# vpc-ccg/tksm

Measured on AMD Instinct MI355X. Metric: sequenced reads/s, higher is better.
Workload: dtype u8; 1 GPU; Bulk molecules, Badread error+qual model (nanopore2020, identity 84,99,5.5), 24 x 128 Mb random genome, FASTQ; kind=bulk, mean_len=1000, length_distribution=normal(1000, 200), compute_qual=True, contexts_in_flight_per_gpu=3

## Files before the change

### tksm_amd/csrc/kernels.h

```cpp
#pragma once
#include <hip/hip_runtime.h>
#include <stdint.h>

namespace tk {

constexpr uint32_t NO_BLOCK = 0xFFFFFFFFu;
constexpr int BLOCK_SHIFT = 12;
constexpr int WAVES_PER_WG = 4;

struct RefView {
    const uint32_t* packed;
    const uint32_t* blocktab;
    const uint8_t* pool;
    const uint64_t* contigs;
    uint32_t n_contigs;
};

struct BatchView {
    const uint32_t* reads;
    const uint32_t* intervals;
    const uint32_t* mods;
    const uint64_t* literals;
    const uint8_t* litpool;
    const uint32_t* ids;
    const uint8_t* idpool;
    uint64_t n_reads;
    uint32_t n_literals;
};

struct ErrModelView {
    int type, k, max_alts;
    int alt0_noop;
    int uniform_nalts;
    const uint32_t* cdf;
    const uint64_t* alts;
    const uint8_t* nalts;
    const uint2* pself2;
    const uint32_t* cdf32;
    const uint4* pseg;
    const uint32_t* pt0;
    const uint4* pt0b;
    const uint4* alts_enc;
};

struct QsModelView {
    int n_slots, kmer_size;
    const uint64_t* keys;
    const uint32_t* row_off;
    const uint32_t* row_cnt;
    const uint32_t* cdf_pool;
    const uint8_t* q_pool;
    const uint4* ent;
    const uint2* pairs;
    const uint8_t* guide;
    int guide_direct;
};

struct IdentView {
    int constant;
    double value;
    const double* qtab;
};

struct TailView {
    int n_lx, n_ly;
    double ratio;
    const double* lx;
    const double* ly;
    const double* cdf;
};
struct TailChain {
    double cum[16];
    uint32_t bases;
    uint32_t pad;
};

struct SimParams {
    uint64_t seed, first_read, stride;
    int mode, compute_q, fastq, quirk_perfect;
    int lcap;
    int ncap;
    int trace_words;
    int s_lcap, s_ncap;
    int ablate;
    int cap_num, cap_den, cap_add;
};

struct SimBuffers {
    const uint32_t* raw_len;
    const uint64_t* slot_off;
    uint8_t* scratch;
    uint32_t* out_len;
    double* identity;
    uint64_t* rec_len;
    uint32_t* status;
    uint32_t* trace;
    unsigned long long* work_counter;
    int32_t* istats;
    double* dstats;
    uint8_t* full_pool; unsigned long long full_pool_bytes; unsigned long long* full_pool_used;
    const uint32_t* tail_len;
    const TailChain* tail_chain;
    uint8_t* big_scratch; size_t big_per_wave; unsigned long long* big_trace;
    const uint32_t* read_list;
    uint64_t n_work;
};

struct ReadState {
    double errors, target, est;
    int32_t change_count;
    uint32_t n_base, aln_no;
    int16_t resume_src, resume_j;
    uint8_t stage;
    uint8_t pending, slow, early;
    int32_t st_draws, st_aligns;
    uint32_t job;
    int32_t raw_len;
    uint32_t res_mt, res_cols, res_fail, pad3;
};

struct RangeGeo {
    uint64_t trace_off;
    uint64_t jc_off;
    uint64_t popd_off;
    uint64_t unused;
    uint32_t tstride;
    uint32_t cw;
    uint32_t ncap;
    uint32_t pad;
};

enum Counter {
    CNT_JOBS = 0,
    CNT_DEFERRED = 1,
    CNT_SLOW = 2,
    CNT_FULL_ROWS = 3,
    CNT_EXIT = 4,
    CNT_REDO_JOBS = 8,
    CNT_REDO_WAVES = 9,
    CNT_REDO_LIST = 10,
    CNT_FAIL = 12,
    CNT_FAIL_OR = 13,
    CNT_FAIL_LAST = 14,
    CNT_FAIL_NM = 15,
    CNT_FAIL_REASON = 16,
    CNT_FAIL_QJOB = 24,
    CNT_FAIL_LIST = 25,
    CNT_EARLY_SLOW = 26,
    CNT_EARLY = 27,
    CNT_WORDS = 32
};
enum ExitCause { EXIT_BAND_LOOP = 0, EXIT_SHIFT_LOOP = 1, EXIT_SHIFT_ERR = 2, EXIT_BAND_ERR = 3 };
enum FailBit { FAIL_QUEUE = 0, FAIL_NOROW = 1, FAIL_SHIFT31 = 3, FAIL_SHIFT14 = 4, FAIL_END_CELL = 5, FAIL_WALK = 6 };

struct FastBuffers {
    ReadState* state;
    const uint32_t* row64;
    uint8_t* st_frag;
    uint16_t* st_nb;
    unsigned long long* st_fplanes;
    uint32_t* st_frag2;
    uint32_t* job_meta;
    uint8_t* job_popd;
    void* trace;
    uint32_t* redo_list;
    void* trace_full;
    uint32_t full_rows, full_tg;
    uint32_t full_cl;
    uint32_t* counters;
    uint32_t* job_cnt;
    uint32_t rs, n_ranges;
    const uint32_t* prev_meta; const uint8_t* prev_popd;
    const uint32_t* prefix;
    const uint32_t* base_cur; const uint32_t* base_prev;
    const RangeGeo* geo_cur; const RangeGeo* geo_prev;
    uint32_t* slow_list;
    uint32_t* early_hist;
    uint2* early_list;
    uint32_t* early_slow;
    uint2* defer_list;
    uint32_t* defer_cnt;
    int defer_len;
};

hipError_t launch_pack(const uint8_t* ascii, uint64_t n, uint64_t gstart, uint32_t* packed, uint32_t* blockflag,
                       hipStream_t s);
hipError_t launch_fill_pool(const uint8_t* ascii, uint64_t n, uint64_t gstart, const uint32_t* blocktab,
                            uint8_t* pool, hipStream_t s);
hipError_t launch_read_lengths(const BatchView& b, const RefView& r, int k, int cap_num, int cap_den, int cap_add,
                               const uint32_t* tail_len, uint32_t* raw_len, uint64_t* slot_cap, uint32_t* status, hipStream_t s);
hipError_t launch_tail_lengths(const BatchView& B, const RefView& R, const TailView& T, uint64_t seed, uint64_t first_read,
                               uint64_t stride, uint32_t* tail_len, hipStream_t s);
hipError_t launch_simulate(const BatchView& b, const RefView& r, const ErrModelView& em, const QsModelView& qm,
                           const IdentView& im, const SimParams& p, const SimBuffers& o, int n_wgs,
                           int waves_per_wg, hipStream_t s);
size_t simulate_big_bytes(int lcap, int ncap);
hipError_t launch_simulate_big(const BatchView& b, const RefView& r, const ErrModelView& em, const QsModelView& qm,
                               const IdentView& im, const SimParams& p, const SimBuffers& o, int n_waves, hipStream_t s);
hipError_t launch_init(const BatchView& b, const RefView& r, const ErrModelView& em, const IdentView& im, const SimParams& p,
                       const SimBuffers& o, const FastBuffers& fb, int waves_per_wg, hipStream_t s);
int err_lds_bytes(int lcap, int ncap, int waves_per_wg, bool state_in_hbm);
int loop_lds_words(int lcap);
hipError_t launch_loopw(const ErrModelView& em, const SimParams& p, const FastBuffers& fb, const uint32_t* order, uint32_t begin,
                        uint32_t count, int lcap, int from_jobs, uint32_t c0, uint32_t c1, hipStream_t s);
hipError_t launch_tail(const ErrModelView& em, const SimParams& p, const FastBuffers& fb, const uint32_t* order, uint32_t begin,
                        uint32_t count, int lcap, int from_jobs, uint32_t c0, uint32_t c1, int wcap, hipStream_t s);
size_t tail_lds_bytes(int lcap);
hipError_t launch_mark_early(const FastBuffers& fb, const uint32_t* order, uint64_t n_reads, int k, uint32_t min_bin, hipStream_t s);
hipError_t launch_tail_early(const ErrModelView& em, const SimParams& p, const FastBuffers& fb, uint32_t max_count, int lcap, int wcap, hipStream_t s);
hipError_t launch_merge_early_slow(const FastBuffers& fb, hipStream_t s);
hipError_t launch_loop(const ErrModelView& em, const SimParams& p, const FastBuffers& fb, const uint32_t* order, uint32_t begin,
                       uint32_t count, int lcap, int from_jobs, uint32_t c0, uint32_t c1, hipStream_t s);
hipError_t launch_err(const BatchView& b, const ErrModelView& em, const QsModelView& qm, const SimParams& p, const SimBuffers& o,
                      const FastBuffers& fb, const uint32_t* order, uint32_t begin, uint32_t count, int lds_lcap, int lds_ncap,
                      int from_jobs, uint32_t c0, uint32_t c1, int waves_per_wg, bool state_in_hbm, hipStream_t s);
hipError_t launch_qjobs(const FastBuffers& fb, int k, uint32_t count, hipStream_t s);
hipError_t launch_round_reset(const FastBuffers& fb, hipStream_t s);
hipError_t launch_collect_unfinished(const FastBuffers& fb, uint64_t n_reads, hipStream_t s);
hipError_t launch_alnf(const SimParams& p, const FastBuffers& fb, const SimBuffers& o, uint32_t n_jobs, bool full_only, int mode, hipStream_t s);
hipError_t launch_perfect_lengths(const BatchView& b, const RefView& r, const SimParams& p, const SimBuffers& o, hipStream_t s);
hipError_t launch_perfect(const BatchView& b, const RefView& r, const SimParams& p, const SimBuffers& o, const uint64_t* rec_off, uint8_t* records,
                          uint32_t max_raw, int n_cus, hipStream_t s);
hipError_t launch_emit(const BatchView& b, const SimParams& p, const SimBuffers& o, const uint64_t* rec_off,
                       uint8_t* records, hipStream_t s);
hipError_t launch_interleave_lens(int n_ranks, const uint64_t* const* offsets, const uint64_t* n_per_rank,
                                  uint64_t n_total, uint64_t* lens, hipStream_t s);
hipError_t launch_interleave_copy(int n_ranks, const uint8_t* const* streams, const uint64_t* const* offsets,
                                  uint64_t n_total, const uint64_t* dst_off, uint8_t* dst, hipStream_t s);
size_t scan_temp_bytes(uint64_t n);
hipError_t launch_scan(const uint64_t* in, uint64_t* out, uint64_t n, void* temp, size_t temp_bytes, hipStream_t s);
hipError_t launch_sum_u32(const uint32_t* in, uint64_t n, unsigned long long* out, hipStream_t s);
int simulate_lds_bytes(int lcap, int ncap, int waves_per_wg);
int simulate_max_wgs(int lds_bytes);

}
```

### tksm_amd/csrc/kernels.hip

```cpp
#include "kernels.h"
#include "loop_filter.h"
#include <type_traits>

namespace tk {

#define DEV __device__ __forceinline__

constexpr int BIG = 1 << 28;
DEV bool is_inf(int v) { return v >= (1 << 27); }

struct Ph4 { uint32_t x, y, z, w; };
enum { ST_ID = 0, ST_PAD = 1, ST_IDENT = 2, ST_DRAW = 3, ST_ALNPOS = 4, ST_QUAL = 5, ST_TAIL = 6 };

DEV Ph4 philox(uint64_t seed, uint64_t read, uint32_t stream, uint32_t n) {
    uint32_t c0 = (uint32_t)read, c1 = (uint32_t)(read >> 32), c2 = stream, c3 = n;
    uint32_t k0 = (uint32_t)seed, k1 = (uint32_t)(seed >> 32);
#pragma unroll
    for (int r = 0; r < 10; r++) {
        const unsigned long long p0 = (unsigned long long)0xD2511F53u * c0, p1 = (unsigned long long)0xCD9E8D57u * c2;
        const uint32_t h0 = (uint32_t)(p0 >> 32), l0 = (uint32_t)p0, h1 = (uint32_t)(p1 >> 32), l1 = (uint32_t)p1;
        uint32_t n0 = h1 ^ c1 ^ k0, n2 = h0 ^ c3 ^ k1;
        c0 = n0; c1 = l1; c2 = n2; c3 = l0;
        k0 += 0x9E3779B9u; k1 += 0xBB67AE85u;
    }
    return Ph4{c0, c1, c2, c3};
}

DEV uint8_t base_char(int code) { return (uint8_t)((0x54474341u >> (8 * (code & 3))) & 0xff); }
DEV int code_of(uint8_t c) { return c == 'A' ? 0 : c == 'C' ? 1 : c == 'G' ? 2 : c == 'T' ? 3 : -1; }
DEV uint8_t upper(uint8_t c) { return (c >= 'a' && c <= 'z') ? (uint8_t)(c - 32) : c; }
DEV uint8_t comp(uint8_t c) {
    return c == 'A' ? 'T' : c == 'C' ? 'G' : c == 'G' ? 'C' : c == 'T' ? 'A' : c;
}

template <int CTRL, int ROW_MASK> DEV int dpp_mov(int old, int src) { return __builtin_amdgcn_update_dpp(old, src, CTRL, ROW_MASK, 0xf, false); }
constexpr int DPP_WAVE_SHL1 = 0x130, DPP_WAVE_SHR1 = 0x138;
#define TKSM_DPP_SCAN(OP, IDENT, x)                         \
    x = OP(x, dpp_mov<0x111, 0xf>(IDENT, x));               \
    x = OP(x, dpp_mov<0x112, 0xf>(IDENT, x));               \
    x = OP(x, dpp_mov<0x114, 0xf>(IDENT, x));               \
    x = OP(x, dpp_mov<0x118, 0xf>(IDENT, x));               \
    x = OP(x, dpp_mov<0x142, 0xa>(IDENT, x));               \
    x = OP(x, dpp_mov<0x143, 0xc>(IDENT, x));
DEV int scan_min_incl(int x, int) { TKSM_DPP_SCAN(min, 0x7fffffff, x) return x; }
DEV int scan_max_incl(int x, int) { TKSM_DPP_SCAN(max, (int)0x80000000, x) return x; }
DEV int add_i32(int a, int b) { return a + b; }
DEV int scan_add_incl(int x, int) { TKSM_DPP_SCAN(add_i32, 0, x) return x; }
DEV uint32_t scan_umax_incl(uint32_t x) {
#define TKSM_UMAX_STEP(C, R) x = max(x, (uint32_t)dpp_mov<C, R>(0, (int)x));
    TKSM_UMAX_STEP(0x111, 0xf) TKSM_UMAX_STEP(0x112, 0xf) TKSM_UMAX_STEP(0x114, 0xf) TKSM_UMAX_STEP(0x118, 0xf) TKSM_UMAX_STEP(0x142, 0xa) TKSM_UMAX_STEP(0x143, 0xc)
#undef TKSM_UMAX_STEP
    return x;
}
DEV int prefix_small(int v, int& total) {
    const unsigned long long b0 = __ballot(v & 1), b1 = __ballot(v & 2), b2 = __ballot(v & 4);
    const int e0 = (int)__builtin_amdgcn_mbcnt_hi((uint32_t)(b0 >> 32), __builtin_amdgcn_mbcnt_lo((uint32_t)b0, 0u));
    const int e1 = (int)__builtin_amdgcn_mbcnt_hi((uint32_t)(b1 >> 32), __builtin_amdgcn_mbcnt_lo((uint32_t)b1, 0u));
    const int e2 = (int)__builtin_amdgcn_mbcnt_hi((uint32_t)(b2 >> 32), __builtin_amdgcn_mbcnt_lo((uint32_t)b2, 0u));
    total = __popcll(b0) + 2 * __popcll(b1) + 4 * __popcll(b2);
    return e0 + 2 * e1 + 4 * e2;
}

DEV void wave_sync() {
    __builtin_amdgcn_fence(__ATOMIC_RELEASE, "wavefront");
    __builtin_amdgcn_wave_barrier();
    __builtin_amdgcn_fence(__ATOMIC_ACQUIRE, "wavefront");
}

DEV uint32_t lo32(unsigned long long v) { return (uint32_t)v; }
DEV uint32_t hi32(unsigned long long v) { return (uint32_t)(v >> 32); }
DEV unsigned long long mk64(uint32_t hi, uint32_t lo) { return ((unsigned long long)hi << 32) | lo; }
DEV uint32_t alignbit(uint32_t hi, uint32_t lo, uint32_t s) { return __builtin_amdgcn_alignbit(hi, lo, s); }
constexpr uint32_t TA = 0xF0u, TB = 0xCCu, TC = 0xAAu;
#define BOOL3(expr) ((uint32_t)((expr) & 0xFFu))
template <uint32_t TT> DEV uint32_t bool3(uint32_t x, uint32_t y, uint32_t z) { return __builtin_amdgcn_bitop3_b32(x, y, z, TT); }
template <uint32_t TT> DEV unsigned long long bool3(unsigned long long x, unsigned long long y, unsigned long long z) {
    return mk64(bool3<TT>(hi32(x), hi32(y), hi32(z)), bool3<TT>(lo32(x), lo32(y), lo32(z)));
}
DEV unsigned long long funnel128(unsigned long long x0, unsigned long long x1, int s) {
    const bool a = (s & 32) != 0;
    const uint32_t b = (uint32_t)s & 31u;
    const uint32_t y0 = a ? hi32(x0) : lo32(x0), y1 = a ? lo32(x1) : hi32(x0), y2 = a ? hi32(x1) : lo32(x1);
    return mk64(alignbit(y2, y1, b), alignbit(y1, y0, b));
}

DEV double sqrt_inrange(double x) {
    const double y = __builtin_amdgcn_rsq(x);
    double g = x * y, h = 0.5 * y;
    const double r = __builtin_fma(-h, g, 0.5);
    g = __builtin_fma(g, r, g); h = __builtin_fma(h, r, h);
    double d = __builtin_fma(-g, g, x);
    g = __builtin_fma(d, h, g);
    d = __builtin_fma(-g, g, x);
    return __builtin_fma(d, h, g);
}
DEV double rcp_refined(double b) {
    double y = __builtin_amdgcn_rcp(b);
    double r = __builtin_fma(-b, y, 1.0);
    y = __builtin_fma(y, r, y);
    r = __builtin_fma(-b, y, 1.0);
    return __builtin_fma(y, r, y);
}
DEV double div_inrange(double a, double b, double yb) {
    const double q = a * yb;
    const double r = __builtin_fma(-b, q, a);
    return __builtin_fma(r, yb, q);
}

DEV uint8_t ref_base(const RefView& R, uint64_t g) {
    uint32_t ex = R.blocktab[g >> BLOCK_SHIFT];
    if (ex != NO_BLOCK) return R.pool[((uint64_t)ex << BLOCK_SHIFT) + (g & ((1u << BLOCK_SHIFT) - 1))];
    uint32_t w = R.packed[g >> 4];
    return base_char((int)(w >> ((g & 15) * 2)));
}

DEV int slot_len(uint32_t code) { return code ? (int)((code >> 12) & 7) : 1; }
DEV uint8_t slot_sym(uint32_t code, int x, uint8_t orig) {
    if (!code) return orig;
    if ((int)((code >> 10) & 3) == x + 1) return orig;
    return base_char((int)(code >> (2 * x)));
}

__global__ void k_pack(const uint8_t* __restrict__ ascii, uint64_t n, uint64_t gstart, uint32_t* __restrict__ packed,
                       uint32_t* __restrict__ blockflag) {
    uint64_t w = (uint64_t)blockIdx.x * blockDim.x + threadIdx.x;
    uint64_t nw = (n + 15) >> 4;
    for (; w < nw; w += (uint64_t)gridDim.x * blockDim.x) {
        uint64_t b0 = w << 4;
        uint32_t word = 0; bool exc = false;
        if (b0 + 16 <= n && ((uintptr_t)(ascii + b0) & 15) == 0) {
            uint4 v = *reinterpret_cast<const uint4*>(ascii + b0);
            uint32_t q[4] = {v.x, v.y, v.z, v.w};
#pragma unroll
            for (int i = 0; i < 16; i++) {
                int c = code_of(upper((uint8_t)(q[i >> 2] >> (8 * (i & 3)))));
                exc |= c < 0; word |= (uint32_t)(c & 3) << (2 * i);
            }
        } else {
            for (int i = 0; i < 16 && b0 + i < n; i++) {
                int c = code_of(upper(ascii[b0 + i]));
                exc |= c < 0; word |= (uint32_t)(c & 3) << (2 * i);
            }
        }
        packed[(gstart >> 4) + w] = word;
        if (exc) blockflag[(gstart + b0) >> BLOCK_SHIFT] = 1;
    }
}

__global__ void k_fill_pool(const uint8_t* __restrict__ ascii, uint64_t n, uint64_t gstart,
                            const uint32_t* __restrict__ blocktab, uint8_t* __restrict__ pool) {
    uint64_t i = (uint64_t)blockIdx.x * blockDim.x + threadIdx.x;
    for (; i < n; i += (uint64_t)gridDim.x * blockDim.x) {
        uint64_t g = gstart + i;
        uint32_t ex = blocktab[g >> BLOCK_SHIFT];
// ... 656 lines not shown
        }
    }
    if (a == 16) {
        uint4 v[4];
#pragma unroll
        for (int q = 0; q < 4; q++) v[q] = c4[4 + q];
#pragma unroll
        for (int q = 0; q < 4; q++) {
            a += !(w < v[q].x) ? 1 : 0; a += !(w < v[q].y) ? 1 : 0; a += !(w < v[q].z) ? 1 : 0; a += !(w < v[q].w) ? 1 : 0;
        }
    }
    return min(a, na);
}

DEV void go_slow(const FastBuffers& FB, uint64_t r, int lane, int cause) {
    if (lane == 0) {
        FB.state[r].slow = 1;
        atomicAdd(&FB.counters[CNT_EXIT + cause], 1u);
        const uint32_t idx = atomicAdd(&FB.counters[CNT_SLOW], 1u);
        FB.slow_list[idx] = (uint32_t)r;
    }
}

DEV uint8_t* frag_row(const FastBuffers& FB, uint64_t r) { return FB.st_frag + (size_t)FB.row64[r] * 64; }
DEV uint16_t* nb_row(const FastBuffers& FB, uint64_t r) { return FB.st_nb + (size_t)FB.row64[r] * 64; }
DEV unsigned long long* planes_row(const FastBuffers& FB, uint64_t r) { return FB.st_fplanes + 2 * ((size_t)FB.row64[r] + 8 * r); }
DEV int planes_words(const FastBuffers& FB, uint64_t r) { return (int)(FB.row64[r + 1] - FB.row64[r]) + 8; }
DEV uint32_t* frag2_row(const FastBuffers& FB, uint64_t r) { return FB.st_frag2 + 4 * ((size_t)FB.row64[r] + r); }
DEV int frag2_words(const FastBuffers& FB, uint64_t r) { return 4 * (int)(FB.row64[r + 1] - FB.row64[r]) + 4; }

DEV uint32_t early_bin(int L, double target) {
    const float sc = (float)L * (float)fmax(0.0, 1.0 - target);
    return (uint32_t)min(255, max(0, (int)(8.0f * __log2f(1.0f + sc))));
}
__global__ __launch_bounds__(256, 7) void k_init(BatchView B, RefView R, ErrModelView EM, IdentView IM, SimParams P,
                                               SimBuffers O, FastBuffers FB) {
#ifndef TKSM_ABLATE
    __builtin_amdgcn_s_setprio(2);
#endif
    const int lane = threadIdx.x & 63, wave = threadIdx.x >> 6, wpw = blockDim.x >> 6;
    const uint64_t r = (uint64_t)blockIdx.x * wpw + wave;
    if (r >= B.n_reads) return;
    uint8_t* frag = lds_raw + (size_t)wave * P.lcap;
    const int k = EM.k;
    const uint64_t g = P.first_read + r * P.stride;
    const int raw_len = (int)O.raw_len[r];
    const int L = raw_len + 2 * k;
    uint32_t status = 0;
    {
        const uint32_t ib = B.reads[2 * r], ic = B.reads[2 * r + 1];
        int o = k;
        for (uint32_t ii = 0; ii < ic; ii++) {
            const Ivl iv = load_interval(B, R, ib + ii);
            const int len = (int)iv.len;
            if (iv.literal) {
                const uint64_t lg = iv.gbase + iv.s;
                for (uint32_t t = (uint32_t)lane; t < (uint32_t)len; t += 64u) {
                    const uint8_t bch = upper(B.litpool[lg + (iv.minus ? (uint32_t)len - 1u - t : t)]);
                    frag[o + t] = iv.minus ? comp(bch) : bch;
                }
            } else
            for (uint32_t t0 = 16u * lane; t0 < (uint32_t)len; t0 += 1024u)
                splice_piece(B, R, iv.gbase + iv.s, (uint32_t)len, false, iv.minus, t0, frag + o + t0);
            wave_sync();
#pragma unroll 1
            for (uint32_t mi = iv.mod_begin; mi < iv.mod_end; mi++) {
                const uint32_t mp = B.mods[2ull * mi], mc = B.mods[2ull * mi + 1];
                if (mp >= (uint32_t)len) { status |= 2; continue; }
                if (lane == 0) frag[o + (iv.minus ? len - 1 - (int)mp : (int)mp)] = iv.minus ? comp((uint8_t)mc) : (uint8_t)mc;
            }
            o += len;
        }
        if (O.tail_len && O.tail_len[r]) tail_fill(O.tail_chain, P.seed, g, frag + o, (int)O.tail_len[r], lane);
    }
    {
        const Ph4 pad = philox(P.seed, g, ST_PAD, 0);
        if (lane < k) {
            frag[lane] = base_char((int)(pad.x >> (2 * lane)));
            frag[k + raw_len + lane] = base_char((int)(pad.y >> (2 * lane)));
        }
    }
    double target;
    if (IM.constant) target = IM.value;
    else {
        const uint32_t u = philox(P.seed, g, ST_IDENT, 0).x;
        const uint32_t idx = u >> 16;
        const double fr = (double)(u & 0xffffu) * (1.0 / 65536.0);
        const double qa = IM.qtab[idx], qb = IM.qtab[idx + 1];
        target = IM.value * (qa + (qb - qa) * fr);
    }
    wave_sync();
    uint8_t* gfrag = frag_row(FB, r);
    unsigned long long* fpl = planes_row(FB, r);
    const int fw_r = planes_words(FB, r), fw2_r = frag2_words(FB, r);
    for (int t = 8 * lane; t < L; t += 512) {
        uint2 c = *reinterpret_cast<const uint2*>(frag + t);
        c.x = ((c.x >> 1) ^ (c.x >> 2)) & 0x03030303u; c.y = ((c.y >> 1) ^ (c.y >> 2)) & 0x03030303u;
        *reinterpret_cast<uint2*>(gfrag + t) = c;
    }
    {
        uint16_t* gnb0 = nb_row(FB, r);
        for (int t = 8 * lane; t < L; t += 512) {
            uint2 c = *reinterpret_cast<const uint2*>(frag + t);
            c.x = ((c.x >> 1) ^ (c.x >> 2)) & 0x03030303u; c.y = ((c.y >> 1) ^ (c.y >> 2)) & 0x03030303u;
            auto two = [](uint32_t b0, uint32_t b1) {
                return (0x1000u | (b0 & 1u) | ((b0 >> 1) << 5)) | ((0x1000u | (b1 & 1u) | ((b1 >> 1) << 5)) << 16);
            };
            uint4 o;
            o.x = two(c.x & 3u, (c.x >> 8) & 3u); o.y = two((c.x >> 16) & 3u, (c.x >> 24) & 3u);
            o.z = two(c.y & 3u, (c.y >> 8) & 3u); o.w = two((c.y >> 16) & 3u, (c.y >> 24) & 3u);
            if (t + 8 > L) {
                const int keep = L - t;
                uint32_t* ow = &o.x;
                for (int x2 = 0; x2 < 8; x2++) if (x2 >= keep) ow[x2 >> 1] &= (x2 & 1) ? 0x0000ffffu : 0xffff0000u;
            }
            *reinterpret_cast<uint4*>(gnb0 + t) = o;
        }
    }
    {
        uint32_t* f2 = frag2_row(FB, r);
        for (int w = lane; w < fw2_r; w += 64) {
            uint32_t word = 0u;
#pragma unroll
            for (int q = 0; q < 4; q++) {
                const int t = 16 * w + 4 * q;
                uint32_t c = t < P.lcap ? *reinterpret_cast<const uint32_t*>(frag + t) : 0u;
                if (t + 4 > L) c = t >= L ? 0u : c & (0xffffffffu >> (8 * (t + 4 - L)));
                const uint32_t codes4 = ((c >> 1) ^ (c >> 2)) & 0x03030303u;
                word |= ((codes4 * 0x40100401u) >> 24) << (24 - 8 * q);
            }
            f2[w] = word;
        }
    }
    bool dirty = false;
    const int nw = (L + 63) >> 6;
    for (int q0 = 0; q0 < fw_r; q0 += 64) {
        unsigned long long mylo = 0ull, myhi = 0ull;
        for (int q = q0; q < min(q0 + 64, nw); q++) {
            const int p = q * 64 + lane;
            const bool valid = p < L;
            const uint8_t c = valid ? frag[p] : (uint8_t)'A';
            const int code = code_of(c);
            dirty |= code < 0;
            const unsigned long long lo = __ballot(valid && (code & 1)), hi = __ballot(valid && (code & 2));
            if (lane == q - q0) { mylo = lo; myhi = hi; }
        }
        if (q0 + lane < fw_r) { ulonglong2 v; v.x = mylo; v.y = myhi; *reinterpret_cast<ulonglong2*>(fpl + 2 * (q0 + lane)) = v; }
    }
    const bool slow = __ballot(dirty) != 0ull;
    if (lane == 0) {
        ReadState S;
        S.errors = 0.0; S.target = target; S.est = 0.0; S.change_count = 0; S.n_base = 0; S.aln_no = 0;
        S.resume_src = -1; S.resume_j = 0; S.stage = 0; S.pending = 0; S.slow = slow ? 1 : 0; S.early = 0;
        S.st_draws = 0; S.st_aligns = 0; S.job = 0; S.raw_len = raw_len; S.res_mt = 0; S.res_cols = 0; S.res_fail = 0; S.pad3 = 0;
        FB.state[r] = S;
        O.status[r] |= status;
        if (slow) { const uint32_t idx = atomicAdd(&FB.counters[CNT_SLOW], 1u); FB.slow_list[idx] = (uint32_t)r; }
        else if (FB.early_hist) atomicAdd(&FB.early_hist[(blockIdx.x & 63u) * 256u + early_bin(L, target)], 1u);
    }
}

DEV void finish_read(const BatchView& B, const SimParams& P, const SimBuffers& O, uint64_t r, int raw_len, int out_len,
                     double identity, uint32_t status, int st_draws, int st_changes, int st_aligns, int L, int st_newlen,
                     int st_strim, int st_etrim, double errors, double target, int lane) {
    if (lane != 0) return;
    if (O.tail_len && !P.quirk_perfect) raw_len -= (int)O.tail_len[r];
    const long long h = pct_hundredths(identity);
    const uint32_t idl = B.ids[2 * r + 1];
    uint64_t rec = 1 + 36 + 8 + ndigits((unsigned)out_len) + 19 + ndigits((unsigned)raw_len) + 15 +
                   ndigits((unsigned long long)(h / 100)) + 3 + 14 + idl + 1;
    rec += (uint64_t)out_len + 1;
    if (P.fastq) rec += 2 + (uint64_t)out_len + 1;
    O.out_len[r] = (uint32_t)out_len;
    O.identity[r] = identity;
    O.rec_len[r] = rec;
    O.status[r] |= status;
    if (O.istats) {
        int32_t* s = O.istats + 16 * r;
        s[0] = st_draws; s[1] = st_changes; s[2] = st_aligns; s[3] = L; s[4] = st_newlen;
        s[5] = st_strim; s[6] = st_etrim; s[7] = (int32_t)status;
        O.dstats[2 * r] = errors; O.dstats[2 * r + 1] = target;
    }
}

DEV uint32_t draw_slot(const uint4& A, int jj) {
    const uint32_t w = (jj >> 1) == 0 ? A.x : (jj >> 1) == 1 ? A.y : (jj >> 1) == 2 ? A.z : A.w;
    return (w >> (16 * (jj & 1))) & 0xffffu;
}

DEV uint32_t planar1(uint32_t a) { return (a & 1u) | ((a >> 1) << 5); }
DEV uint32_t planar2(uint32_t a, uint32_t b) { return (a & 1u) | ((b & 1u) << 1) | ((a >> 1) << 5) | ((b >> 1) << 6); }
DEV uint4 random_change_enc(int kidx, int k, uint32_t type, uint32_t pos, uint32_t base4, uint32_t side, uint32_t r3) {
    uint32_t e[8];
#pragma unroll
    for (int j = 0; j < 8; j++) {
        const uint32_t kc = j < k ? (uint32_t)(kidx >> (2 * (k - 1 - j))) & 3u : 0u;
        uint32_t v = (1u << 12) | planar1(kc);
        if ((uint32_t)j == pos)
            v = type == 0 ? 0x8000u | (1u << 12) | planar1((kc + r3) & 3u)
              : type == 1 ? 0x8000u | (2u << 12) | (side ? planar2(kc, base4) : planar2(base4, kc))
                          : 0x8000u;
        e[j] = j < k ? v : 0u;
    }
    return make_uint4(e[0] | (e[1] << 16), e[2] | (e[3] << 16), e[4] | (e[5] << 16), e[6] | (e[7] << 16));
}

struct SlotEval { uint32_t am, lens; uint32_t e[4]; };
DEV SlotEval eval_draw(const uint16_t* nb, int k, int i, const uint4& A, bool acc) {
    SlotEval r;
    r.am = 0; r.lens = 0;
    r.e[0] = A.x | 0x80008000u; r.e[1] = A.y | 0x80008000u; r.e[2] = A.z | 0x80008000u; r.e[3] = A.w | 0x80008000u;
    if (acc) {
#pragma unroll
        for (int jj = 0; jj < 8; jj++) {
            if (jj < k) {
                const uint32_t e = draw_slot(A, jj);
                if ((e >> 15) && (nb[i + jj] & 0x8000u) == 0) r.am |= 1u << jj;
                r.lens |= ((e >> 12) & 7u) << (3 * jj);
            }
        }
    }
    return r;
}

DEV int joined_len(const uint16_t* nb, int p0, int n, int lane) {
    int m = 0;
    for (int q = 0; q < n; q += 64) {
        const int p = q + lane;
        const int len = p < n ? slot_len(nb[p0 + p]) : 0;
        int total;
        (void)prefix_small(len, total);
        m += total;
    }
    return m;
}

DEV void join_out(const uint8_t* frag, const uint16_t* nb, int n, uint8_t* out_seq, int lo, int hi, int lane) {
    int base = 0;
    for (int q = 0; q < n; q += 64) {
        const int p = q + lane;
        uint32_t code = 0; int len = 0; uint8_t orig = 0;
        if (p < n) { code = nb[p]; len = slot_len(code); orig = frag[p]; }
        int total;
        const int off = base + prefix_small(len, total);
        const uint32_t syms = code ? code & 0x3ffu : planar1((uint32_t)orig);
        for (int x2 = 0; x2 < len; x2++) { const int c = off + x2; if (c >= lo && c < hi) out_seq[c - lo] = base_char((int)(((syms >> x2) & 1u) | (((syms >> (5 + x2)) & 1u) << 1))); }
        base += total;
    }
}

#ifndef TKSM_LOOP_N
#define TKSM_LOOP_N 16
#define TKSM_LOOP_K 3
#endif
constexpr int LOOP_N = TKSM_LOOP_N, LOOP_K = TKSM_LOOP_K;
__global__ __launch_bounds__(64) __attribute__((amdgpu_num_vgpr(128))) void k_loop(ErrModelView EM, SimParams P, FastBuffers FB, const uint32_t* __restrict__ order,
                                              uint32_t begin, uint32_t count, int Wl, int from_jobs, uint32_t c0, uint32_t c1) {
#ifndef TKSM_ABLATE
    __builtin_amdgcn_s_setprio(2);
#endif
    uint32_t* lf = reinterpret_cast<uint32_t*>(lds_raw);
    const int lane = threadIdx.x;
    const uint32_t widx = blockIdx.x * 64u + (uint32_t)lane;
    bool act = widx < count;
    uint32_t r = 0, rc = 0;
    if (act) {
        if (!from_jobs) { r = order[begin + widx]; rc = (begin + widx) / FB.rs; }
        else {
            const uint32_t target = FB.prefix[c0] + widx;
            uint32_t lo2 = c0, hi2 = c1 - 1;
            while (lo2 < hi2) { const uint32_t mid = (lo2 + hi2 + 1) >> 1; if (FB.prefix[mid] <= target) lo2 = mid; else hi2 = mid - 1; }
            r = FB.prev_meta[4ull * (FB.base_prev[lo2] + (target - FB.prefix[lo2]))];
            rc = lo2;
        }
    }
    ReadState* sp = FB.state + r;
    ReadState S{};
    if (act) S = *sp;
    act = act && S.stage == 0 && !S.slow && !S.early;
    const int k = EM.k;
    const int L = S.raw_len + 2 * k;
    const uint32_t* f2 = frag2_row(FB, r);
    for (int w = 0; w < Wl; w += 16) {
        uint4 v[4];
#pragma unroll
        for (int q = 0; q < 4; q++) v[q] = *reinterpret_cast<const uint4*>(f2 + min(w + 4 * q, Wl - 4));
#pragma unroll
        for (int q = 0; q < 4; q++) {
            const int ww = min(w + 4 * q, Wl - 4);
            lf[(ww + 0) * 64 + lane] = v[q].x; lf[(ww + 1) * 64 + lane] = v[q].y; lf[(ww + 2) * 64 + lane] = v[q].z; lf[(ww + 3) * 64 + lane] = v[q].w;
        }
    }
    uint32_t* lfb = lf + (size_t)Wl * 64;
    {
        uint4 v[4];
#pragma unroll
        for (int q = 0; q < 4; q++) v[q] = EM.pt0b[q * 64 + lane];
#pragma unroll
        for (int q = 0; q < 4; q++) *reinterpret_cast<uint4*>(lfb + 4 * (q * 64 + lane)) = v[q];
    }
    __syncthreads();
    const uint16_t* lfe = reinterpret_cast<const uint16_t*>(lfb);
    uint16_t* gnb = nb_row(FB, r);
    const uint64_t g = P.first_read + (uint64_t)r * P.stride;
    const double frag_len = (double)L, target = S.target;
    const double rcp_len = rcp_refined(act ? frag_len : 1.0);
    double errors = S.errors;
    int change_count = S.change_count;
    uint32_t n = S.n_base, aln_no = S.aln_no;
    int resume_j = S.resume_j, st_draws = S.st_draws;
    double est_keep = S.est;
    if (act && S.pending == 1) {
        const uint32_t mt = S.res_mt, cols = S.res_cols;
        if (S.res_fail) {
            sp->slow = 1;
            atomicAdd(&FB.counters[CNT_EXIT + EXIT_BAND_LOOP], 1u);
            FB.slow_list[atomicAdd(&FB.counters[CNT_SLOW], 1u)] = r;
            act = false;
        } else {
            const double ident = cols ? (double)mt / (double)cols : 0.0;
            if (L <= 1000) errors = (1.0 - ident) * frag_len;
            else {
                const double estimated = (1.0 - ident) * frag_len;
                const double weight = 1000.0 / frag_len;
                errors = estimated * weight + errors * (1.0 - weight);
            }
            aln_no++;
        }
    }
    const uint32_t kmer_range = (uint32_t)(L - k);
    const long long loop_limit = 100ll * L;
    const uint32_t kmask = (1u << (2 * k)) - 1u;
    int cc25 = change_count % 25;
    enum { RUN = 0, NEED_ALN = 1, DONE = 2, IDLE = 3 };
    int st = act ? RUN : IDLE;
#ifdef TKSM_ABLATE
    if (P.ablate == 33) st = IDLE;
#endif
    const bool use_tab = EM.type != 0 && EM.alt0_noop;
    while (__ballot(st == RUN) != 0ull) {
        if (st != RUN) continue;
        const uint32_t navail = (uint32_t)max(0ll, min((long long)LOOP_N, loop_limit - (long long)n));
        uint32_t mask = 0u;
        {
            uint32_t dwv[LOOP_N], kxv[LOOP_N];
#pragma unroll
            for (int b = 0; b < LOOP_N; b++) {
                const Ph4 d = philox(P.seed, g, ST_DRAW, n + (uint32_t)b);
                const int di1 = (int)__umulhi(d.x, kmer_range);
                dwv[b] = d.y;
                const int w = di1 >> 4, o = di1 & 15;
#ifdef TKSM_ABLATE
                const bool abl_lds = P.ablate == 35 || P.ablate == 36;
                const uint32_t hi = (abl_lds || w < Wl) ? lf[min(w, Wl - 1) * 64 + lane] : f2[w], lo = (abl_lds || w + 1 < Wl) ? lf[min(w + 1, Wl - 1) * 64 + lane] : f2[w + 1];
#else
                const uint32_t hi = w < Wl ? lf[w * 64 + lane] : f2[w], lo = w + 1 < Wl ? lf[(w + 1) * 64 + lane] : f2[w + 1];
#endif
                kxv[b] = (uint32_t)(mk64(hi, lo) >> (64 - 2 * o - 2 * k)) & kmask;
            }
            uint32_t ev[LOOP_N];
#pragma unroll
            for (int b = 0; b < LOOP_N; b++) ev[b] = lfe[tklf::loop_filter_key(kxv[b])];
            uint32_t sure = 0u, und = 0u;
#pragma unroll
            for (int b = 0; b < LOOP_N; b++) {
                const int c = tklf::loop_filter_classify(ev[b], dwv[b]);
                sure |= c == tklf::DRAW_CHANGE ? 1u << b : 0u;
                und |= c == tklf::DRAW_UNDECIDED ? 1u << b : 0u;
            }
            if (!use_tab) { sure = (1u << LOOP_N) - 1u; und = 0u; }
#ifdef TKSM_ABLATE
            const bool abl_t0 = P.ablate == 34 || P.ablate == 36;
            if (abl_t0 && use_tab) { sure = 0u; und = (1u << LOOP_N) - 1u; }
#endif
            uint32_t t0v[LOOP_N];
#pragma unroll
            for (int b = 0; b < LOOP_N; b++) {
                const uint32_t off = (und >> b) & 1u ? kxv[b] << 2 : 0u;
#ifdef TKSM_ABLATE
                t0v[b] = abl_t0 ? 0xCF000000u : *reinterpret_cast<const uint32_t*>(reinterpret_cast<const char*>(EM.pt0) + off);
#else
                t0v[b] = *reinterpret_cast<const uint32_t*>(reinterpret_cast<const char*>(EM.pt0) + off);
#endif
            }
#pragma unroll
            for (int b = 0; b < LOOP_N; b++) mask |= !(dwv[b] < t0v[b]) ? 1u << b : 0u;
            mask = (sure | (und & mask)) & ((1u << navail) - 1u);
        }
        int di[LOOP_K], kidx[LOOP_K];
        uint32_t bj[LOOP_K], dw[LOOP_K];
        bool rest;
        {
            uint32_t mm = mask;
#pragma unroll
            for (int j = 0; j < LOOP_K; j++) {
                bj[j] = mm ? (uint32_t)__builtin_ctz(mm) : (uint32_t)LOOP_N;
                mm &= mm - 1u;
                const uint32_t bb = min(bj[j], (uint32_t)LOOP_N - 1u);
                const Ph4 d = philox(P.seed, g, ST_DRAW, n + bb);
                dw[j] = d.y;
                di[j] = (int)__umulhi(d.x, kmer_range);
                const int w = di[j] >> 4, o = di[j] & 15;
                const uint32_t hi = w < Wl ? lf[w * 64 + lane] : f2[w], lo = w + 1 < Wl ? lf[(w + 1) * 64 + lane] : f2[w + 1];
                kidx[j] = (int)((uint32_t)(mk64(hi, lo) >> (64 - 2 * o - 2 * k)) & kmask);
            }
            rest = mm != 0u;
        }
        int cls[LOOP_K];
        uint4 seg[LOOP_K];
        int nab[LOOP_K];
#pragma unroll
        for (int j = 0; j < LOOP_K; j++) { seg[j] = EM.pseg[kidx[j]]; nab[j] = EM.max_alts; }
        if (!EM.uniform_nalts) {
#pragma unroll
            for (int j = 0; j < LOOP_K; j++) nab[j] = (int)EM.nalts[kidx[j]];
        }
        int sbase[LOOP_K];
        uint4 th0[LOOP_K], th1[LOOP_K];
        struct __attribute__((packed, aligned(4))) W5 { uint32_t v[5]; };
        W5 nbw[LOOP_K];
#pragma unroll
        for (int j = 0; j < LOOP_K; j++) {
            const bool have = bj[j] < (uint32_t)LOOP_N;
            cls[j] = !have ? 0 : EM.type == 0 ? 2 : (dw[j] < seg[j].x ? (EM.alt0_noop ? 0 : 3) : 1);
            sbase[j] = 8 * ((dw[j] < seg[j].y ? 0 : 1) + (dw[j] < seg[j].z ? 0 : 1) + (dw[j] < seg[j].w ? 0 : 1));
            const uint4* c4 = reinterpret_cast<const uint4*>(EM.cdf32 + (cls[j] == 1 ? (size_t)kidx[j] * 32 + sbase[j] : (size_t)0));
            th0[j] = c4[0]; th1[j] = c4[1];
            const uint16_t* gp = cls[j] != 0 ? gnb + (di[j] & ~1) : FB.st_nb;
            nbw[j] = *reinterpret_cast<const W5*>(gp);
        }
        uint4 alt[LOOP_K];
#pragma unroll
        for (int j = 0; j < LOOP_K; j++) {
            size_t at = 0;
            if (cls[j] == 1 || cls[j] == 3) {
                const int na = nab[j];
                int a2 = 0;
                if (cls[j] == 1) {
                    const uint32_t w = dw[j];
                    a2 = sbase[j];
                    a2 += !(w < th0[j].x) ? 1 : 0; a2 += !(w < th0[j].y) ? 1 : 0; a2 += !(w < th0[j].z) ? 1 : 0; a2 += !(w < th0[j].w) ? 1 : 0;
                    a2 += !(w < th1[j].x) ? 1 : 0; a2 += !(w < th1[j].y) ? 1 : 0; a2 += !(w < th1[j].z) ? 1 : 0; a2 += !(w < th1[j].w) ? 1 : 0;
                    a2 = min(a2, na);
                }
                if (a2 == na) cls[j] = 2;
                else if (a2 == 0 && EM.alt0_noop) cls[j] = 0;
                else at = (size_t)kidx[j] * EM.max_alts + a2;
            }
            alt[j] = EM.alts_enc[at];
        }
        const uint32_t n0 = n;
        const uint32_t end = rest ? bj[LOOP_K - 1] + 1u : navail;
        uint32_t wrote = 0u;
        auto top_of_iteration = [&](double& est) -> bool {
            est = 1.0 - div_inrange(errors, frag_len, rcp_len);
            if ((double)change_count > 0.9 * frag_len || est <= target) { st = DONE; st_draws = (int)n; return false; }
            if ((long long)n + 1 > loop_limit) { st = DONE; st_draws = (int)loop_limit; return false; }
            return true;
        };
#pragma unroll
        for (int j = 0; j <= LOOP_K; j++) {
            if (st != RUN) break;
            double est = est_keep;
            if (j == LOOP_K || bj[j] >= (uint32_t)LOOP_N) {
                if (n - n0 < end) { if (!top_of_iteration(est)) break; n = n0 + end; }
                if (!rest && navail < (uint32_t)LOOP_N) (void)top_of_iteration(est);
                break;
            }
            if (resume_j == 0 && !top_of_iteration(est)) break;
            n = n0 + bj[j];
            if (cls[j] != 0) {
                uint4 A = alt[j];
                if (cls[j] == 2) {
                    const Ph4 d2 = philox(P.seed, g, ST_DRAW, n0 + bj[j]);
                    const uint32_t dzj = d2.z, dvj = d2.w;
                    const uint32_t type = __umulhi(dzj, 3u), pos = __umulhi(dvj, (uint32_t)k);
                    const uint32_t base4 = dvj & 3u, side = (dvj >> 2) & 1u;
                    const uint32_t r3 = (((dzj & 0xffffu) * 3u) >> 16) + 1u;
                    const uint32_t kc = ((uint32_t)kidx[j] >> (2 * (k - 1 - (int)pos))) & 3u;
                    const uint32_t v = type == 0 ? 0x8000u | (1u << 12) | planar1((kc + r3) & 3u)
                                     : type == 1 ? 0x8000u | (2u << 12) | (side ? planar2(kc, base4) : planar2(base4, kc))
                                                 : 0x8000u;
                    const uint32_t w = v << (16 * (pos & 1u)), which = pos >> 1;
                    A = make_uint4(which == 0 ? w : 0u, which == 1 ? w : 0u, which == 2 ? w : 0u, which == 3 ? w : 0u);
                }
                uint32_t dm = ((A.x >> 15) & 1u) | ((A.x >> 31) << 1) | (((A.y >> 15) & 1u) << 2) | ((A.y >> 31) << 3) |
                              (((A.z >> 15) & 1u) << 4) | ((A.z >> 31) << 5) | (((A.w >> 15) & 1u) << 6) | ((A.w >> 31) << 7);
                dm &= ((1u << k) - 1u) & ~((1u << resume_j) - 1u);
                if (dm) {
                    bool stale = false;
#pragma unroll
                    for (int j2 = 0; j2 < LOOP_K; j2++) if (j2 < j) stale |= ((wrote >> j2) & 1u) && abs(di[j] - di[j2]) < k;
                    if (stale) nbw[j] = *reinterpret_cast<const W5*>(gnb + (di[j] & ~1));
                    const double f15 = est * sqrt_inrange(est);
                    const int odd = di[j] & 1;
                    int stop_at = -1;
                    while (dm) {
                        const int jj = __builtin_ctz(dm);
                        dm &= dm - 1u;
                        const int ent = jj + odd, wi = ent >> 1;
                        const uint32_t cw2 = wi == 0 ? nbw[j].v[0] : wi == 1 ? nbw[j].v[1] : wi == 2 ? nbw[j].v[2] : wi == 3 ? nbw[j].v[3] : nbw[j].v[4];
                        if (((cw2 >> (16 * (ent & 1))) & 0x8000u) == 0u) {
                            const uint32_t e = draw_slot(A, jj);
                            gnb[di[j] + jj] = (uint16_t)(e | 0x8000u);
                            wrote |= 1u << j;
                            change_count++;
                            const int len_j = (int)((e >> 12) & 7u);
                            errors += (double)(len_j < 2 ? 1 : len_j - 1) * f15;
                            if (++cc25 == 25) { cc25 = 0; stop_at = jj; dm = 0u; }
                        }
                    }
                    if (stop_at >= 0) {
                        st = NEED_ALN;
                        if (stop_at + 1 < k) { resume_j = stop_at + 1; est_keep = est; }
                        else { resume_j = 0; n++; }
                        break;
                    }
                }
            }
            resume_j = 0;
            n++;
        }
    }
    int st_aligns = S.st_aligns;
    uint32_t job = 0;
    {
        bool need = st == NEED_ALN;
        unsigned long long todo = __ballot(need);
        while (todo) {
            const int leader = __builtin_ctzll(todo);
            const uint32_t lrc = (uint32_t)__shfl((int)rc, leader, 64);
            const unsigned long long grp = __ballot(need && rc == lrc);
            uint32_t base = 0;
            if (lane == leader) base = FB.base_cur[lrc] + atomicAdd(&FB.job_cnt[lrc * 32u], (uint32_t)__popcll(grp));
            base = (uint32_t)__shfl((int)base, leader, 64);
            if (need && rc == lrc) { job = base + (uint32_t)__popcll(grp & ((1ull << lane) - 1ull)); need = false; }
            todo &= ~grp;
        }
    }
    if (st == NEED_ALN) {
        st_aligns++;
        uint32_t p0 = 0, nrows = (uint32_t)L;
        if (L > 1000) {
            uint32_t r2 = r;
            asm volatile("" : "+v"(r2));
            p0 = __umulhi(philox(P.seed, P.first_read + (uint64_t)r2 * P.stride, ST_ALNPOS, aln_no).x, (uint32_t)(L - 1000 + 1));
            nrows = 1000u;
        }
        *reinterpret_cast<uint4*>(FB.job_meta + 4ull * job) = make_uint4(r, p0, nrows, 0u);
    }
    if (st == NEED_ALN || st == DONE) {
        sp->errors = errors; sp->est = est_keep; sp->change_count = change_count; sp->n_base = n; sp->aln_no = aln_no;
        sp->resume_src = -1; sp->resume_j = (int16_t)resume_j; sp->st_draws = st_draws; sp->st_aligns = st_aligns;
        sp->pending = st == NEED_ALN ? 1 : 0;
        sp->job = job;
        sp->stage = st == NEED_ALN ? 0 : 3;
        if (st == DONE) {
            atomicAdd(&FB.defer_cnt[rc * 32u], 1u);
            FB.defer_list[atomicAdd(&FB.counters[CNT_DEFERRED], 1u)] = make_uint2(r, rc);
        }
    }
}

constexpr int TAIL_WCAP = 2048, TAIL_FCAP = 1024;
__host__ __device__ inline size_t tail_bitmap_bytes(int lcap) { return ((size_t)((lcap + 63) / 64) * 8 + 16 + 15) & ~(size_t)15; }
DEV int join_window_planar(const uint16_t* gnb, int p0, int n, uint8_t* N, uint16_t* owner, int ncap, int lane) {
    uint32_t codes[16];
#pragma unroll
    for (int q = 0; q < 16; q++) codes[q] = 64 * q + lane < n ? (uint32_t)gnb[p0 + 64 * q + lane] : 0u;
    int base = 0;
#pragma unroll
    for (int q = 0; q < 16; q++) {
        if (64 * q >= n) break;
        const int p = 64 * q + lane;
        const uint32_t code = codes[q];
        const int len = (int)((code >> 12) & 7u);
        int total;
        const int off = base + prefix_small(len, total);
        if (off + len <= ncap)
            for (int x2 = 0; x2 < len; x2++) {
                N[off + x2] = (uint8_t)(((code >> x2) & 1u) | (((code >> (5 + x2)) & 1u) << 1));
                owner[off + x2] = (uint16_t)p;
            }
        base += total;
    }
    return base;
}
template <bool TAIL>
__global__ __launch_bounds__(64) void k_loopw(ErrModelView EM, SimParams P, FastBuffers FB, const uint32_t* __restrict__ order,
                                               uint32_t begin, uint32_t count, int from_jobs, uint32_t c0, uint32_t c1, int lcap, int wcap) {
    uint16_t* nbl = reinterpret_cast<uint16_t*>(lds_raw);
    uint32_t* bml = reinterpret_cast<uint32_t*>(lds_raw);
    uint8_t* Fw = lds_raw + tail_bitmap_bytes(lcap);
    uint8_t* Nw = Fw + TAIL_FCAP;
    uint16_t* ownw = reinterpret_cast<uint16_t*>(Nw + TAIL_WCAP);
    const int lane = threadIdx.x;
    const uint32_t widx = blockIdx.x;
    if (widx >= count) return;
    uint32_t r, rc;
#ifndef TKSM_ABLATE
    if (TAIL) __builtin_amdgcn_s_setprio(3);
#ifndef TKSM_ABLATE
    if (!TAIL) __builtin_amdgcn_s_setprio(2);
#endif
#endif
    const bool early_mode = TAIL && from_jobs == 3;
    if (early_mode) {
        if (widx >= FB.counters[CNT_EARLY]) return;
        const uint2 e = FB.early_list[widx];
        r = e.x; rc = e.y;
    } else if (!from_jobs) { r = order[begin + widx]; rc = (begin + widx) / FB.rs; }
    else {
        const uint32_t target = FB.prefix[c0] + widx;
        uint32_t lo2 = c0, hi2 = c1 - 1;
        while (lo2 < hi2) { const uint32_t mid = (lo2 + hi2 + 1) >> 1; if (FB.prefix[mid] <= target) lo2 = mid; else hi2 = mid - 1; }
        r = FB.prev_meta[4ull * (FB.base_prev[lo2] + (target - FB.prefix[lo2]))];
        rc = lo2;
    }
    r = (uint32_t)__builtin_amdgcn_readfirstlane((int)r); rc = (uint32_t)__builtin_amdgcn_readfirstlane((int)rc);
    ReadState* sp = FB.state + r;
    const ReadState S = *sp;
    if (S.stage != 0 || S.slow || (S.early && !early_mode)) return;
    auto to_exact_kernel = [&]() {
        if (!early_mode) { go_slow(FB, r, lane, EXIT_BAND_LOOP); return; }
        if (lane == 0) { sp->slow = 1; FB.early_slow[atomicAdd(&FB.counters[CNT_EARLY_SLOW], 1u)] = r; }
    };
    const int k = EM.k;
    const int L = S.raw_len + 2 * k;
    const uint32_t* f2 = frag2_row(FB, r);
    uint16_t* gnb = nb_row(FB, r);
    if (!TAIL) {
        for (int t = 2 * lane; t < L; t += 128) *reinterpret_cast<uint32_t*>(nbl + t) = *reinterpret_cast<const uint32_t*>(gnb + t);
    } else {
        for (int t = 32 * lane; t < L; t += 2048) {
            const uint4* c4 = reinterpret_cast<const uint4*>(gnb + t);
            uint32_t word = 0u;
#pragma unroll
            for (int q = 0; q < 4; q++) {
                const uint4 v = c4[q];
                const uint32_t w4[4] = {v.x, v.y, v.z, v.w};
#pragma unroll
                for (int e = 0; e < 4; e++) word |= (((w4[e] >> 15) & 1u) | ((w4[e] >> 31) << 1)) << (8 * q + 2 * e);
            }
            bml[t >> 5] = word;
        }
    }
    wave_sync();
    const uint64_t g = P.first_read + (uint64_t)r * P.stride;
    const double frag_len = (double)L, target = S.target;
    const double rcp_len = rcp_refined(frag_len);
    double errors = S.errors;
    int change_count = S.change_count;
    uint32_t n = S.n_base, aln_no = S.aln_no;
    int resume_j = S.resume_j, st_draws = S.st_draws;
    double est_keep = S.est;
    if (S.pending == 1) {
        if (S.res_fail) {
            if (lane == 0) {
                sp->slow = 1;
                atomicAdd(&FB.counters[CNT_EXIT + EXIT_BAND_LOOP], 1u);
                FB.slow_list[atomicAdd(&FB.counters[CNT_SLOW], 1u)] = r;
            }
            return;
        }
        const uint32_t mt = S.res_mt, cols = S.res_cols;
        const double ident = cols ? (double)mt / (double)cols : 0.0;
        if (L <= 1000) errors = (1.0 - ident) * frag_len;
        else {
            const double estimated = (1.0 - ident) * frag_len;
            const double weight = 1000.0 / frag_len;
            errors = estimated * weight + errors * (1.0 - weight);
        }
        aln_no++;
    }
    const uint32_t kmer_range = (uint32_t)(L - k);
    const long long loop_limit = 100ll * L;
    const uint32_t kmask = (1u << (2 * k)) - 1u;
    int cc25 = change_count % 25;
    enum { RUN = 0, NEED_ALN = 1, DONE = 2 };
    int st = RUN;
    int st_aligns = S.st_aligns;
    const uint8_t* gfrag = frag_row(FB, r);
    if (TAIL && L <= 1000) { for (int t = lane; t < L; t += 64) Fw[t] = gfrag[t]; }
    for (;;) {
        while (st == RUN) {
            double est_cur = est_keep;
            if (resume_j == 0) {
                est_cur = 1.0 - div_inrange(errors, frag_len, rcp_len);
                if ((double)change_count > 0.9 * frag_len || est_cur <= target) { st = DONE; st_draws = (int)n; break; }
            }
            const uint32_t nl = n + (uint32_t)lane;
            const bool live = (long long)nl + 1 <= loop_limit;
            const Ph4 d = philox(P.seed, g, ST_DRAW, nl);
            const int di = (int)__umulhi(d.x, kmer_range);
            const int w = di >> 4, o = di & 15;
            const int kidx = (int)((uint32_t)(mk64(f2[w], f2[w + 1]) >> (64 - 2 * o - 2 * k)) & kmask);
            const uint4 seg = EM.pseg[kidx];
            const int na = EM.uniform_nalts ? EM.max_alts : (int)EM.nalts[kidx];
            int cls = EM.type == 0 ? 2 : (d.y < seg.x ? (EM.alt0_noop ? 0 : 3) : 1);
            const int sbase = 8 * ((d.y < seg.y ? 0 : 1) + (d.y < seg.z ? 0 : 1) + (d.y < seg.w ? 0 : 1));
            const uint4* c4 = reinterpret_cast<const uint4*>(EM.cdf32 + (cls == 1 ? (size_t)kidx * 32 + sbase : (size_t)0));
            const uint4 th0 = c4[0], th1 = c4[1];
            size_t at = 0;
            if (cls == 1 || cls == 3) {
                int a = 0;
                if (cls == 1) {
// ... 1365 lines not shown
```

Baseline: 15.60 million reads/s.

## Keep a persistent queue of classified draws across k_loop iterations

Replaces the per-iteration mask of classified draws with a 64-bit queue that carries leftover classified draws to the next iteration, and saves it in ReadState across alignment pauses. The k_loop iteration only generates and classifies a new batch of LOOP_N Philox draws when the queue has room. This avoids re-computing Philox draws and filter classifications that an earlier iteration already did but did not consume. It adds queue bookkeeping, extra state (a new dq field in ReadState), and more complex control flow that may cost registers under the 128-VGPR cap.

```diff
diff --git a/tksm_amd/csrc/kernels.h b/tksm_amd/csrc/kernels.h
--- a/tksm_amd/csrc/kernels.h
+++ b/tksm_amd/csrc/kernels.h
@@ -1,5 +1,6 @@
 #pragma once
 #include <hip/hip_runtime.h>
+#include <stddef.h>
 #include <stdint.h>
 
 namespace tk {
@@ -116,8 +117,10 @@
     int32_t st_draws, st_aligns;
     uint32_t job;
     int32_t raw_len;
-    uint32_t res_mt, res_cols, res_fail, pad3;
-};
+    uint32_t res_mt, res_cols, res_fail;
+    uint64_t dq;
+};
+static_assert(sizeof(ReadState) == 80 && offsetof(ReadState, dq) == 72 && offsetof(ReadState, res_mt) == 60, "ReadState layout");
 
 struct RangeGeo {
     uint64_t trace_off;
diff --git a/tksm_amd/csrc/kernels.hip b/tksm_amd/csrc/kernels.hip
--- a/tksm_amd/csrc/kernels.hip
+++ b/tksm_amd/csrc/kernels.hip
@@ -1,5 +1,6 @@
 #include "kernels.h"
 #include "loop_filter.h"
+#include "loop_queue.h"
 #include <type_traits>
 
 namespace tk {
@@ -962,7 +963,7 @@
         ReadState S;
         S.errors = 0.0; S.target = target; S.est = 0.0; S.change_count = 0; S.n_base = 0; S.aln_no = 0;
         S.resume_src = -1; S.resume_j = 0; S.stage = 0; S.pending = 0; S.slow = slow ? 1 : 0; S.early = 0;
-        S.st_draws = 0; S.st_aligns = 0; S.job = 0; S.raw_len = raw_len; S.res_mt = 0; S.res_cols = 0; S.res_fail = 0; S.pad3 = 0;
+        S.st_draws = 0; S.st_aligns = 0; S.job = 0; S.raw_len = raw_len; S.res_mt = 0; S.res_cols = 0; S.res_fail = 0; S.dq = 0;
         FB.state[r] = S;
         O.status[r] |= status;
         if (slow) { const uint32_t idx = atomicAdd(&FB.counters[CNT_SLOW], 1u); FB.slow_list[idx] = (uint32_t)r; }
@@ -1063,7 +1064,13 @@
 #define TKSM_LOOP_N 16
 #define TKSM_LOOP_K 3
 #endif
+__device__ __forceinline__ uint32_t bit_below(uint32_t m, bool c) {
+    m = (m << 1) | (c ? 1u : 0u);
+    asm volatile("" : "+v"(m));
+    return m;
+}
 constexpr int LOOP_N = TKSM_LOOP_N, LOOP_K = TKSM_LOOP_K;
+static_assert(tklq::refill_fits(LOOP_N) && LOOP_K >= 1, "TKSM_LOOP_N must be 1 .. 31 and at most the width of k_loop's queue of classified draws");
 __global__ __launch_bounds__(64) __attribute__((amdgpu_num_vgpr(128))) void k_loop(ErrModelView EM, SimParams P, FastBuffers FB, const uint32_t* __restrict__ order,
                                               uint32_t begin, uint32_t count, int Wl, int from_jobs, uint32_t c0, uint32_t c1) {
 #ifndef TKSM_ABLATE
@@ -1119,6 +1126,9 @@
     int change_count = S.change_count;
     uint32_t n = S.n_base, aln_no = S.aln_no;
     int resume_j = S.resume_j, st_draws = S.st_draws;
+    tklq::qword dq;
+    uint32_t cnt;
+    tklq::queue_restore(S.resume_src, S.dq, dq, cnt);
     double est_keep = S.est;
     if (act && S.pending == 1) {
         const uint32_t mt = S.res_mt, cols = S.res_cols;
@@ -1150,13 +1160,14 @@
     const bool use_tab = EM.type != 0 && EM.alt0_noop;
     while (__ballot(st == RUN) != 0ull) {
         if (st != RUN) continue;
-        const uint32_t navail = (uint32_t)max(0ll, min((long long)LOOP_N, loop_limit - (long long)n));
-        uint32_t mask = 0u;
-        {
+        const bool room = tklq::queue_has_room(cnt, LOOP_N);
+        if (__ballot(room) != 0ull) {
+            const uint32_t nq = n + cnt;
+            uint32_t mask = 0u;
             uint32_t dwv[LOOP_N], kxv[LOOP_N];
 #pragma unroll
             for (int b = 0; b < LOOP_N; b++) {
-                const Ph4 d = philox(P.seed, g, ST_DRAW, n + (uint32_t)b);
+                const Ph4 d = philox(P.seed, g, ST_DRAW, nq + (uint32_t)b);
                 const int di1 = (int)__umulhi(d.x, kmer_range);
                 dwv[b] = d.y;
                 const int w = di1 >> 4, o = di1 & 15;
@@ -1173,10 +1184,10 @@
             for (int b = 0; b < LOOP_N; b++) ev[b] = lfe[tklf::loop_filter_key(kxv[b])];
             uint32_t sure = 0u, und = 0u;
 #pragma unroll
-            for (int b = 0; b < LOOP_N; b++) {
+            for (int b = LOOP_N - 1; b >= 0; b--) {
                 const int c = tklf::loop_filter_classify(ev[b], dwv[b]);
-                sure |= c == tklf::DRAW_CHANGE ? 1u << b : 0u;
-                und |= c == tklf::DRAW_UNDECIDED ? 1u << b : 0u;
+                sure = bit_below(sure, c == tklf::DRAW_CHANGE);
+                und = bit_below(und, c == tklf::DRAW_UNDECIDED);
             }
             if (!use_tab) { sure = (1u << LOOP_N) - 1u; und = 0u; }
 #ifdef TKSM_ABLATE
@@ -1194,19 +1205,16 @@
 #endif
             }
 #pragma unroll
-            for (int b = 0; b < LOOP_N; b++) mask |= !(dwv[b] < t0v[b]) ? 1u << b : 0u;
-            mask = (sure | (und & mask)) & ((1u << navail) - 1u);
+            for (int b = LOOP_N - 1; b >= 0; b--) mask = bit_below(mask, !(dwv[b] < t0v[b]));
+            tklq::queue_append(dq, cnt, sure | (und & mask), room ? tklq::queue_refill_count(n, cnt, loop_limit, LOOP_N) : 0u);
         }
         int di[LOOP_K], kidx[LOOP_K];
         uint32_t bj[LOOP_K], dw[LOOP_K];
-        bool rest;
+        const bool rest = tklq::queue_choose<LOOP_K>(dq, bj);
         {
-            uint32_t mm = mask;
 #pragma unroll
             for (int j = 0; j < LOOP_K; j++) {
-                bj[j] = mm ? (uint32_t)__builtin_ctz(mm) : (uint32_t)LOOP_N;
-                mm &= mm - 1u;
-                const uint32_t bb = min(bj[j], (uint32_t)LOOP_N - 1u);
+                const uint32_t bb = min(bj[j], tklq::NO_DRAW - 1u);
                 const Ph4 d = philox(P.seed, g, ST_DRAW, n + bb);
                 dw[j] = d.y;
                 di[j] = (int)__umulhi(d.x, kmer_range);
@@ -1214,7 +1222,6 @@
                 const uint32_t hi = w < Wl ? lf[w * 64 + lane] : f2[w], lo = w + 1 < Wl ? lf[(w + 1) * 64 + lane] : f2[w + 1];
                 kidx[j] = (int)((uint32_t)(mk64(hi, lo) >> (64 - 2 * o - 2 * k)) & kmask);
             }
-            rest = mm != 0u;
         }
         int cls[LOOP_K];
         uint4 seg[LOOP_K];
@@ -1231,7 +1238,7 @@
         W5 nbw[LOOP_K];
 #pragma unroll
         for (int j = 0; j < LOOP_K; j++) {
-            const bool have = bj[j] < (uint32_t)LOOP_N;
+            const bool have = bj[j] != tklq::NO_DRAW;
             cls[j] = !have ? 0 : EM.type == 0 ? 2 : (dw[j] < seg[j].x ? (EM.alt0_noop ? 0 : 3) : 1);
             sbase[j] = 8 * ((dw[j] < seg[j].y ? 0 : 1) + (dw[j] < seg[j].z ? 0 : 1) + (dw[j] < seg[j].w ? 0 : 1));
             const uint4* c4 = reinterpret_cast<const uint4*>(EM.cdf32 + (cls[j] == 1 ? (size_t)kidx[j] * 32 + sbase[j] : (size_t)0));
@@ -1260,7 +1267,7 @@
             alt[j] = EM.alts_enc[at];
         }
         const uint32_t n0 = n;
-        const uint32_t end = rest ? bj[LOOP_K - 1] + 1u : navail;
+        const uint32_t end = tklq::queue_end(rest, bj[LOOP_K - 1], cnt);
         uint32_t wrote = 0u;
         auto top_of_iteration = [&](double& est) -> bool {
             est = 1.0 - div_inrange(errors, frag_len, rcp_len);
@@ -1272,9 +1279,9 @@
         for (int j = 0; j <= LOOP_K; j++) {
             if (st != RUN) break;
             double est = est_keep;
-            if (j == LOOP_K || bj[j] >= (uint32_t)LOOP_N) {
+            if (j == LOOP_K || bj[j] == tklq::NO_DRAW) {
                 if (n - n0 < end) { if (!top_of_iteration(est)) break; n = n0 + end; }
-                if (!rest && navail < (uint32_t)LOOP_N) (void)top_of_iteration(est);
+                if (!rest && tklq::queue_at_limit(n0, cnt, loop_limit)) (void)top_of_iteration(est);
                 break;
             }
             if (resume_j == 0 && !top_of_iteration(est)) break;
@@ -1331,6 +1338,7 @@
             resume_j = 0;
             n++;
         }
+        tklq::queue_consume(dq, cnt, n - n0);
     }
     int st_aligns = S.st_aligns;
     uint32_t job = 0;
@@ -1361,7 +1369,9 @@
     }
     if (st == NEED_ALN || st == DONE) {
         sp->errors = errors; sp->est = est_keep; sp->change_count = change_count; sp->n_base = n; sp->aln_no = aln_no;
-        sp->resume_src = -1; sp->resume_j = (int16_t)resume_j; sp->st_draws = st_draws; sp->st_aligns = st_aligns;
+        sp->resume_src = st == NEED_ALN ? tklq::queue_saved_count(cnt) : (int16_t)tklq::NO_QUEUE;
+        if (st == NEED_ALN) sp->dq = dq;
+        sp->resume_j = (int16_t)resume_j; sp->st_draws = st_draws; sp->st_aligns = st_aligns;
         sp->pending = st == NEED_ALN ? 1 : 0;
         sp->job = job;
         sp->stage = st == NEED_ALN ? 0 : 3;
diff --git a/tksm_amd/csrc/loop_queue.h b/tksm_amd/csrc/loop_queue.h
--- /dev/null
+++ b/tksm_amd/csrc/loop_queue.h
@@ -0,0 +1,72 @@
+#pragma once
+#include <stdint.h>
+
+#if defined(__HIPCC__)
+#define TKLQ_HD __host__ __device__ inline
+#else
+#define TKLQ_HD inline
+#endif
+
+#ifndef TKLQ_BITS
+#define TKLQ_BITS 64
+#endif
+
+namespace tklq {
+
+constexpr int QUEUE_BITS = TKLQ_BITS;
+static_assert(QUEUE_BITS == 32 || QUEUE_BITS == 64, "the queue is one machine word");
+#if TKLQ_BITS == 64
+typedef uint64_t qword;
+TKLQ_HD uint32_t first_set(qword m) { return (uint32_t)__builtin_ctzll(m); }
+#else
+typedef uint32_t qword;
+TKLQ_HD uint32_t first_set(qword m) { return (uint32_t)__builtin_ctz(m); }
+#endif
+constexpr uint32_t NO_DRAW = (uint32_t)QUEUE_BITS;
+constexpr int NO_QUEUE = -1;
+
+constexpr bool refill_fits(int refill) { return refill >= 1 && refill < 32 && refill <= QUEUE_BITS; }
+
+TKLQ_HD bool queue_has_room(uint32_t cnt, int refill) { return cnt + (uint32_t)refill <= (uint32_t)QUEUE_BITS; }
+
+TKLQ_HD uint32_t queue_refill_count(uint32_t n, uint32_t cnt, long long limit, int refill) {
+    const long long left = limit - ((long long)n + (long long)cnt);
+    return (uint32_t)(left < 0 ? 0 : (left < (long long)refill ? left : (long long)refill));
+}
+
+TKLQ_HD void queue_append(qword& dq, uint32_t& cnt, uint32_t bits, uint32_t nav) {
+    const uint32_t sh = nav ? cnt : 0u;
+    dq |= (qword)(bits & ((1u << nav) - 1u)) << sh;
+    cnt += nav;
+}
+
+template <int K>
+TKLQ_HD bool queue_choose(qword dq, uint32_t (&bj)[K]) {
+    qword mm = dq;
+#if defined(__HIPCC__)
+#pragma unroll
+#endif
+    for (int j = 0; j < K; j++) {
+        bj[j] = mm ? first_set(mm) : NO_DRAW;
+        mm &= mm - 1u;
+    }
+    return mm != 0u;
+}
+
+TKLQ_HD uint32_t queue_end(bool rest, uint32_t bj_last, uint32_t cnt) { return rest ? bj_last + 1u : cnt; }
+
+TKLQ_HD bool queue_at_limit(uint32_t n, uint32_t cnt, long long limit) { return (long long)n + (long long)cnt >= limit; }
+
+TKLQ_HD void queue_consume(qword& dq, uint32_t& cnt, uint32_t c) {
+    dq = c >= (uint32_t)QUEUE_BITS ? (qword)0 : dq >> c;
+    cnt -= c;
+}
+
+TKLQ_HD int16_t queue_saved_count(uint32_t cnt) { return (int16_t)cnt; }
+TKLQ_HD void queue_restore(int saved_cnt, uint64_t saved_dq, qword& dq, uint32_t& cnt) {
+    const bool have = saved_cnt > 0 && saved_cnt <= QUEUE_BITS;
+    cnt = have ? (uint32_t)saved_cnt : 0u;
+    dq = have ? (qword)saved_dq : (qword)0;
+}
+
+}
```

Result: no change. 15.68 million reads/s (median of 4 runs) (+0.5%).
